# pratikvn/schwarz-lib

Hardware: AMD Instinct MI355X
Metric: RAS iterations/sec + time-to-residual(1e-6), 3D Poisson, 1/2/4/8 subdomains (higher is better)
Workload: dtype f64; 1 GPU; 3D Poisson 256^3, 1 subdomain on 1 MI355X (BASELINE configs[1]); inner_cg_iters=10, precond=jacobi, overlap=2, partition=regular, rows_per_gpu=16777216, nnz_per_gpu=117047296, spmv_variant=0, matrix_format=row-pair coded, cg_flavour=254, exchange=two-sided, all-gathered residual norms

## Files before the change

### schwarz-lib_amd/csrc/spmv_pair.hip

```cpp
#include <hip/hip_runtime.h>

#include <algorithm>
#include <cstdlib>
#include <cstring>
#include <unordered_map>
#include <vector>

#include "device_utils.hpp"
#include "schwz_hip.h"
#include "schwz_internal.hpp"

namespace schwz {

constexpr int kPairPats = 64;
constexpr int kPairEntries = 512;
constexpr int kPairChunk = 8;
constexpr int kPairTableLds = kPairEntries * 16 + kPairEntries * 4 + (kPairEntries / 4) * 4;

__host__ __device__ inline int pair_stride(int lmax, int ch = kPairChunk) { return (lmax + ch - 1) / ch * ch; }

struct __attribute__((aligned(16))) PairVal {
    double a, b;
};
struct __attribute__((aligned(8))) PairMeta {
// ... 421 lines not shown
            } else {
                accumulate(a.x, ra, base, len, safe, s0, s1, own, own_from_gathers);
                if (dual_t) accumulate(a.x2, ra, base, len, safe, t0, t1, unused, false);
            }
        } else {
            plain_row(ra, dual_t, s0, t0);
            if (has_b) plain_row(ra + 1, dual_t, s1, t1);
        }
        if (kWantOwn && !own_from_gathers) {
            own.x = kDir ? dir1(ra) : a.x[ra];
            if (has_b) own.y = kDir ? dir1(ra + 1) : a.x[ra + 1];
        }
        double y0, y1 = 0.0, p0, p1 = 0.0;
        finish(ra, s0, t0, dual_t, own.x, ob0, od0, y0, p0);
        if (has_b) finish(ra + 1, s1, t1, dual_t, own.y, ob1, od1, y1, p1);
        if (MODE == kSpmvCgUpdate) {
            if (has_b) {
                const pvd2 rr = {y0, y1};
                const pvd2 xx = {cgx.x + p0, cgx.y + p1};
                __builtin_nontemporal_store(rr, reinterpret_cast<pvd2 *>(a.cg_r + ra));
                if (a.cg_x) __builtin_nontemporal_store(xx, reinterpret_cast<pvd2 *>(a.cg_x + ra));
            } else {
                a.cg_r[ra] = y0;
                if (a.cg_x) a.cg_x[ra] = cgx.x + p0;
            }
        } else if (kDir) {
            if (has_b)
                __builtin_memcpy(a.y + ra, &own, 16);
            else
                a.y[ra] = own.x;
        } else if (MODE != kSpmvResidNorm && !kDotOnly) {
            if (has_b) {
                const pvd2 yy = {y0, y1};
                if (MODE == kSpmvResidInit || MODE == kSpmvResidDual)
                    __builtin_nontemporal_store(yy, reinterpret_cast<pvd2 *>(a.y + ra));
                else
                    __builtin_memcpy(a.y + ra, &yy, 16);
            } else {
                a.y[ra] = y0;
            }
        }
        if (MODE == kSpmvResidInit || MODE == kSpmvResidDual) {
            if (has_b) {
                const pvd2 pp = {p0, p1};
                __builtin_nontemporal_store(pp, reinterpret_cast<pvd2 *>(a.p + ra));
            } else {
                a.p[ra] = p0;
            }
        }
    }
    if (MODE != kSpmvPlain) {
        const double s0 = block_sum(acc0, red);
        const double s1 = block_sum(acc1, red);
        if (tid == 0) {
            const int stride = a.part_stride ? a.part_stride : (int)gridDim.x;
            a.partials[a.part_offset + blockIdx.x] = s0;
            a.partials[stride + a.part_offset + blockIdx.x] = s1;
        }
        if (MODE == kSpmvResidDual) {
            const double s2v = block_sum(acc2, red);
            if (tid == 0) a.partials[2 * gridDim.x + blockIdx.x] = s2v;
        }
    }
    if (kDir && blockIdx.x == 0 && tid == 0 && !a.sweep) {
        CgState *st = const_cast<CgState *>(a.cg_state);
        st->rho[(a.it + 1) & 1] = cg_rho_new;
        st->rr = cg_rr;
        st->iters = st->iters + 1;
        if (sqrt(cg_rr) <= a.cg_rtol * st->r0) st->stop_iter = 0;
    }
}

#ifndef SCHWZ_WALK_ZEROCOEF
#define SCHWZ_WALK_ZEROCOEF 1
#endif

#ifndef SCHWZ_WALK_HINTS
#define SCHWZ_WALK_HINTS 1
#endif
#ifndef SCHWZ_INIT_PLAIN_STORE
#define SCHWZ_INIT_PLAIN_STORE 1
#endif

template <int NHL, int NH, bool DIAGVEC, bool INIT = false, bool DUAL = false, int RUNS = 8>
__global__ __launch_bounds__(kBlock) void spmv_pair_sweep_kernel(CsrView A, SpmvArgs a)
{
#pragma clang fp contract(off)
    extern __shared__ __attribute__((aligned(16))) char sweep_lds[];
    constexpr int T = NH * kPairRows;
    const int NX = A.sweep_nx;
    double *const own_ring = reinterpret_cast<double *>(sweep_lds);
    double *const halo_ring = own_ring + 4 * T;
    PairVal *const cpv = reinterpret_cast<PairVal *>(halo_ring + 4 * NX);
    int *const cmask = reinterpret_cast<int *>(cpv + A.canon_npat * 9);
    __shared__ double red[4];
    double cg_alpha = 1.0;
    const int tid = threadIdx.x;
    if (!INIT) {
        if (a.it >= a.cg_state->stop_iter) return;
    }
    typedef double pvd2u __attribute__((ext_vector_type(2), aligned(8)));
    const double *const r_in = INIT ? a.b : a.cg_r;
    double *const r_out = INIT ? a.y : (a.cg_r_out ? a.cg_r_out : a.cg_r);
    const pvd2 ring_scale = {a.ring_scale, a.ring_scale};
    auto tables_and_alpha = [&]() {
        for (int i = tid; i < A.canon_npat * 9; i += kBlock) {
            if (SCHWZ_WALK_ZEROCOEF) {
                const int m = A.canon_mask[i / 9], k = i % 9;
                cpv[i] = PairVal{((m >> k) & 1) ? A.canon_val[2 * i] : 0.0, ((m >> (16 + k)) & 1) ? A.canon_val[2 * i + 1] : 0.0};
            } else {
                cpv[i] = PairVal{A.canon_val[2 * i], A.canon_val[2 * i + 1]};
            }
        }
        if (tid < A.canon_npat) cmask[tid] = A.canon_mask[tid];
        if (!INIT) {
            cg_alpha = a.cg_state->rho[a.it & 1] / fold_partials(a.pq_partials, a.pq_nparts, red);
            if (blockIdx.x == 0 && tid == 0 && a.alpha_out) *a.alpha_out = cg_alpha;
        }
        lds_barrier();
    };
    if (blockIdx.x == 0)
        for (int i = (int)gridDim.x + a.part_offset + tid; i < a.part_stride; i += kBlock) {
            a.partials[i] = a.partials[a.part_stride + i] = 0.0;
            if (DUAL) a.partials[2 * a.part_stride + i] = 0.0;
        }
    const int4 sg = A.sweep_seg[blockIdx.x];
    const int64_t PL = A.sweep_pl;
    const int band = sg.x, z0 = sg.y, z1 = sg.z;
    constexpr bool GEN = RUNS == 0;
    const int blen = GEN ? sg.w : T;
    const int64_t gmax = A.ncols - 2;
    double acc0 = 0.0, acc1 = 0.0, acc2 = 0.0;
    typedef const unsigned __attribute__((address_space(4))) *const_words;
    typedef const int __attribute__((address_space(4))) *const_ints;
    if (z0 < z1) {
        const const_ints chain = (const_ints)(uintptr_t)A.chain_plane;
        const const_ints chain_far = (const_ints)(uintptr_t)A.chain_far;
        auto band_row = [&](int z) -> int {
            const int k = chain[z];
            return (k < 0 ? 0 : k) * (int)PL + band * T;
        };
        auto clampg = [&](int g) -> int { return g < 0 ? 0 : (g > (int)gmax ? (int)gmax : g); };
        auto load_own = [&](int base, pvd2 (&reg)[NH]) {
#pragma unroll
            for (int k = 0; k < NH; ++k) __builtin_memcpy(&reg[k], a.x + clampg(base + 2 * (tid + k * kBlock)), 16);
        };
        auto store_own = [&](int z, const pvd2 (&reg)[NH]) {
            double *slot_p = own_ring + (size_t)(z & 3) * T;
#pragma unroll
            for (int k = 0; k < NH; ++k) *reinterpret_cast<pvd2 *>(slot_p + 2 * (tid + k * kBlock)) = ring_scale * reg[k];
        };
        auto load_halo = [&](int base, pvd2 (&reg)[NHL]) {
            const int lo = base - NX, up = base + T;
#pragma unroll
            for (int k = 0; k < NHL; ++k) {
                const int pc = min(tid + k * kBlock, NX - 1);
                const int g = pc < NX / 2 ? lo + 2 * pc : up + 2 * (pc - NX / 2);
                __builtin_memcpy(&reg[k], a.x + clampg(g), 16);
            }
        };
        auto store_halo = [&](int z, const pvd2 (&reg)[NHL]) {
            double *slot_p = halo_ring + (size_t)(z & 1) * 2 * NX;
#pragma unroll
            for (int k = 0; k < NHL; ++k) {
                const int pc = min(tid + k * kBlock, NX - 1);
                *reinterpret_cast<pvd2 *>(slot_p + 2 * pc) = ring_scale * reg[k];
            }
        };
        struct Ahead {
            pvd2 r, d;
            unsigned w[GEN ? 1 : RUNS / 2];
        };
        auto fetch = [&](int base, int h) -> Ahead {
            Ahead f;
            const int row0 = base + h * kPairRows;
            const int ra = GEN ? base + min(h * kPairRows + 2 * tid, blen - 2) : row0 + 2 * tid;
            if (GEN) {
                f.w[0] = A.pair_id[ra >> 1];
            } else {
                const const_words q = (const_words)(uintptr_t)(A.pair_rle + (row0 / kPairRows) * ((RUNS ? RUNS : 8) / 8));
#pragma unroll
                for (int k = 0; k < (GEN ? 1 : RUNS / 2); ++k) f.w[k] = q[k];
            }
            if (SCHWZ_WALK_HINTS)
                f.r = __builtin_nontemporal_load(reinterpret_cast<const pvd2u *>(r_in + ra));
            else
                f.r = *reinterpret_cast<const pvd2u *>(r_in + ra);
            if (DIAGVEC) f.d = __builtin_nontemporal_load(reinterpret_cast<const pvd2 *>(a.dinv + ra));
            return f;
        };
        pvd2 own_a[NH], own_b[NH], hreg[NHL];
        Ahead r_a[NH], r_b[NH];
        int brow[5];
#pragma unroll
        for (int k = 0; k < 5; ++k) brow[k] = band_row(z0 - 1 + k);
        {
            pvd2 first[NH], second[NH];
            load_own(brow[0], first);
            load_own(brow[1], second);
            load_halo(brow[1], hreg);
            load_own(brow[2], own_b);
            load_own(brow[3], own_a);
#pragma unroll
            for (int h = 0; h < NH; ++h) {
                r_a[h] = fetch(brow[1], h);
                r_b[h] = fetch(z0 + 1 < z1 ? brow[2] : brow[1], h);
            }
            tables_and_alpha();
            store_own(z0 - 1, first);
            store_own(z0, second);
        }
        auto step = [&](int z, pvd2 (&own_next)[NH], Ahead (&rr)[NH]) {
            store_own(z + 1, own_next);
            store_halo(z, hreg);
            lds_barrier();
            load_halo(brow[2], hreg);
            load_own(brow[4], own_next);
            const int far = chain_far[z];
            const bool plain_pos = DUAL ? ((const_ints)(uintptr_t)A.chain_dual)[z] == 0 : true;
            const double *cur = own_ring + (size_t)(z & 3) * T;
            const double *prv = own_ring + (size_t)((z + 3) & 3) * T;
            const double *nxt = own_ring + (size_t)((z + 1) & 3) * T;
            const double *hlo = halo_ring + (size_t)(z & 1) * 2 * NX, *hup = hlo + NX;
            const double *fb0 = (far & 3) == 1 ? prv : ((far & 3) == 2 ? nxt : cur);
            const double *fb1 = ((far >> 2) & 3) == 1 ? prv : (((far >> 2) & 3) == 2 ? nxt : cur);
            const double *fa0 = ((far >> 4) & 3) == 1 ? prv : (((far >> 4) & 3) == 2 ? nxt : cur);
            const double *fa1 = ((far >> 6) & 3) == 1 ? prv : (((far >> 6) & 3) == 2 ? nxt : cur);
            const int rbase = z + 2 < z1 ? brow[3] : brow[1];
#pragma unroll
            for (int h = 0; h < NH; ++h) {
                const Ahead f = rr[h];
                const int i0u = h * kPairRows + 2 * tid;
                const bool valid = !GEN || i0u < blen;
                const int i0 = GEN ? min(i0u, blen - 2) : i0u;
                const int ra = brow[1] + i0;
                int pid = GEN ? (int)f.w[0] : (int)((f.w[0] >> 8) & 0xffu);
#pragma unroll
                for (int k = 1; k < RUNS; ++k) {
                    const unsigned e = (f.w[k >> 1] >> ((k & 1) * 16)) & 0xffffu;
                    if ((unsigned)tid >= (e & 0xffu)) pid = (int)(e >> 8);
                }
                const int mask = SCHWZ_WALK_ZEROCOEF ? 0 : cmask[pid];
                pvd2 t[8];
                t[4] = *reinterpret_cast<const pvd2 *>(cur + i0);
                t[3].x = i0 > 0 ? cur[i0 - 1] : hlo[NX - 1];
                t[3].y = t[4].x;
                t[5].x = t[4].y;
                t[5].y = i0 + 2 < T ? cur[i0 + 2] : hup[0];
                t[2] = *reinterpret_cast<const pvd2 *>(i0 >= NX ? cur + (i0 - NX) : hlo + i0);
                t[6] = *reinterpret_cast<const pvd2 *>(i0 + NX < T ? cur + (i0 + NX) : hup + (i0 + NX - T));
                t[0] = *reinterpret_cast<const pvd2 *>(fb0 + i0);
                t[7] = *reinterpret_cast<const pvd2 *>(fa0 + i0);
                double s0 = 0.0, s1 = 0.0;
                auto add = [&](int k, pvd2 tv) {
                    const PairVal v = cpv[pid * 9 + k];
                    const double p0 = v.a * tv.x, p1 = v.b * tv.y;
                    if (SCHWZ_WALK_ZEROCOEF) {
                        s0 += p0;
                        s1 += p1;
                    } else {
                        s0 += ((mask >> k) & 1) ? p0 : 0.0;
                        s1 += ((mask >> (16 + k)) & 1) ? p1 : 0.0;
                    }
                };
                add(0, t[0]);
                if (far & 0x0c) add(1, *reinterpret_cast<const pvd2 *>(fb1 + i0));
#pragma unroll
                for (int k = 2; k < 8; ++k) add(k, t[k]);
                if (far & 0xc0) add(8, *reinterpret_cast<const pvd2 *>(fa1 + i0));
                const double r0 = INIT ? f.r.x - s0 : f.r.x - cg_alpha * s0;
                const double zz0 = a.diag_mode ? (DIAGVEC ? f.d.x : a.diag_uniform) * r0 : r0;
                const double r1 = INIT ? f.r.y - s1 : f.r.y - cg_alpha * s1;
                const double zz1 = a.diag_mode ? (DIAGVEC ? f.d.y : a.diag_uniform) * r1 : r1;
                if (GEN) {
                    const double t00 = r0 * zz0, t01 = r0 * r0, t10 = r1 * zz1, t11 = r1 * r1;
                    acc0 += valid ? t00 : 0.0;
                    acc1 += valid ? t01 : 0.0;
                    acc0 += valid ? t10 : 0.0;
                    acc1 += valid ? t11 : 0.0;
                } else {
                    acc0 += r0 * zz0;
                    acc1 += r0 * r0;
                    acc0 += r1 * zz1;
                    acc1 += r1 * r1;
                }
                if (DUAL) {
                    const double q0 = r0 * r0, q1 = r1 * r1;
                    acc2 += plain_pos ? q0 : 0.0;
                    acc2 += plain_pos ? q1 : 0.0;
                }
                const pvd2 rn = {r0, r1};
                if (SCHWZ_WALK_HINTS && !(INIT && SCHWZ_INIT_PLAIN_STORE))
                    __builtin_nontemporal_store(rn, reinterpret_cast<pvd2 *>(r_out + ra));
                else
                    *reinterpret_cast<pvd2 *>(r_out + ra) = rn;
                rr[h] = fetch(rbase, h);
            }
#pragma unroll
            for (int k = 0; k < 4; ++k) brow[k] = brow[k + 1];
            brow[4] = band_row(z + 4);
        };
        int z = z0;
        for (; z + 1 < z1; z += 2) {
            step(z, own_b, r_a);
            step(z + 1, own_a, r_b);
        }
        if (z < z1) step(z, own_b, r_a);
    } else if (!INIT && blockIdx.x == 0) {
        tables_and_alpha();
    }
    const double s0 = block_sum(acc0, red);
    const double s1 = block_sum(acc1, red);
    if (tid == 0) {
        a.partials[blockIdx.x] = s0;
        a.partials[a.part_stride + blockIdx.x] = s1;
    }
    if (DUAL) {
        const double s2 = block_sum(acc2, red);
        if (tid == 0) a.partials[2 * a.part_stride + blockIdx.x] = s2;
    }
}

#ifndef SCHWZ_DD
#define SCHWZ_DD 7
#endif
template <int NHL, int NH, bool FIRST = false, int RUNS = 8>
__global__ __launch_bounds__(kBlock) void spmv_pair_dirdot_sweep_kernel(CsrView A, SpmvArgs a)
{
#pragma clang fp contract(off)
    extern __shared__ __attribute__((aligned(16))) char sweep_lds[];
    constexpr int T = NH * kPairRows;
    const int NX = A.sweep_nx;
    double *const own_ring = reinterpret_cast<double *>(sweep_lds);
    constexpr int kHaloSlots = (SCHWZ_DD & 2) ? 3 : 2;
    double *const halo_ring = own_ring + 4 * T;
    PairVal *const cpv = reinterpret_cast<PairVal *>(halo_ring + kHaloSlots * NX);
    int *const cmask = reinterpret_cast<int *>(cpv + A.canon_npat * 5);
    __shared__ double red[4];
    if (!FIRST && a.it >= a.cg_state->stop_iter) return;
    double cg_rho_new = 0.0, cg_rr = 0.0, cg_beta = 0.0;
    const int tid = threadIdx.x;
    auto init_fold = [&]() {
        if (FIRST && a.init_fold && blockIdx.x == 0)
            cg_init_state(const_cast<CgState *>(a.cg_state), a.pq_partials, a.pq_nparts, a.cg_rtol, a.norm_sq_out,
                          a.norm_bank, red);
    };
    auto tables_and_beta = [&]() {
        for (int i = tid; i < A.canon_npat * 5; i += kBlock) {
            if (SCHWZ_WALK_ZEROCOEF) {
                const int m = A.canon_sym_mask[i / 5], k = i % 5;
                cpv[i] = PairVal{((m >> k) & 1) ? A.canon_sym_val[2 * i] : 0.0, ((m >> (16 + k)) & 1) ? A.canon_sym_val[2 * i + 1] : 0.0};
            } else {
                cpv[i] = PairVal{A.canon_sym_val[2 * i], A.canon_sym_val[2 * i + 1]};
            }
        }
        if (tid < A.canon_npat) cmask[tid] = A.canon_sym_mask[tid];
        if (!FIRST) {
            cg_rho_new = fold_partials(a.pq_partials, a.pq_nparts, red);
            cg_rr = fold_partials(a.pq_partials + a.pq_nparts, a.pq_nparts, red);
            cg_beta = cg_rho_new / a.cg_state->rho[a.it & 1];
        }
        init_fold();
        lds_barrier();
    };
    if (blockIdx.x == 0)
        for (int i = (int)gridDim.x + a.part_offset + tid; i < a.part_stride; i += kBlock)
            a.partials[i] = a.partials[a.part_stride + i] = 0.0;
    const int4 sg = A.sweep_seg_dir[blockIdx.x];
    const int64_t PL = A.sweep_pl;
    const int band = sg.x, z0 = sg.y, z1 = sg.z;
    constexpr bool GEN = RUNS == 0;
    const int blen = GEN ? sg.w : T;
    const int64_t gmax = A.ncols - 2;
    const pvd2 du = {a.diag_uniform, a.diag_uniform};
    double acc0 = 0.0;
    typedef const unsigned __attribute__((address_space(4))) *const_words;
    typedef const int __attribute__((address_space(4))) *const_ints;
    if (z0 < z1) {
        const const_ints chain = (const_ints)(uintptr_t)A.chain_plane;
        const const_ints chain_far = (const_ints)(uintptr_t)A.chain_far;
        auto band_row = [&](int z) -> int {
            const int k = chain[z];
            return (k < 0 ? 0 : k) * (int)PL + band * T;
        };
        auto clampg = [&](int g) -> int { return g < 0 ? 0 : (g > (int)gmax ? (int)gmax : g); };
        const pvd2 p_scale = {a.p_scale, a.p_scale};
        auto newp = [&](pvd2 rv, pvd2 pv) -> pvd2 {
            const pvd2 zv = a.diag_mode ? du * rv : rv;
            if (FIRST) return zv;
            const pvd2 ps = p_scale * pv;
// ... 119 lines not shown
            const double *prv = own_ring + (size_t)((z + 3) & 3) * T;
            const double *nxt = own_ring + (size_t)((z + 1) & 3) * T;
            const double *hup = halo_ring + (size_t)((SCHWZ_DD & 2) ? hs : (z & 1)) * NX;
            const double *fa0 = ((far >> 4) & 3) == 1 ? prv : (((far >> 4) & 3) == 2 ? nxt : cur);
            const double *fa1 = ((far >> 6) & 3) == 1 ? prv : (((far >> 6) & 3) == 2 ? nxt : cur);
            const int rbase = z + 2 < z1 ? brow[3] : brow[1];
#pragma unroll
            for (int h = 0; h < NH; ++h) {
                const Rle f = rl[h];
                const int i0u = h * kPairRows + 2 * tid;
                const bool valid = !GEN || i0u < blen;
                const int i0 = GEN ? min(i0u, blen - 2) : i0u;
                int pid = GEN ? (int)f.w[0] : (int)((f.w[0] >> 8) & 0xffu);
#pragma unroll
                for (int k = 1; k < RUNS; ++k) {
                    const unsigned e = (f.w[k >> 1] >> ((k & 1) * 16)) & 0xffffu;
                    if ((unsigned)tid >= (e & 0xffu)) pid = (int)(e >> 8);
                }
                const int mask = SCHWZ_WALK_ZEROCOEF ? 0 : cmask[pid];
                pvd2 t[4];
                t[0] = *reinterpret_cast<const pvd2 *>(cur + i0);
                t[1].x = t[0].y;
                t[1].y = i0 + 2 < T ? cur[i0 + 2] : hup[0];
                t[2] = *reinterpret_cast<const pvd2 *>(i0 + NX < T ? cur + (i0 + NX) : hup + (i0 + NX - T));
                t[3] = *reinterpret_cast<const pvd2 *>(fa0 + i0);
                double s0 = 0.0, s1 = 0.0;
                auto add = [&](int k, pvd2 tv) {
                    const PairVal v = cpv[pid * 5 + k];
                    const double p0 = v.a * tv.x, p1 = v.b * tv.y;
                    if (SCHWZ_WALK_ZEROCOEF) {
                        s0 += p0;
                        s1 += p1;
                    } else {
                        s0 += ((mask >> k) & 1) ? p0 : 0.0;
                        s1 += ((mask >> (16 + k)) & 1) ? p1 : 0.0;
                    }
                };
#pragma unroll
                for (int k = 0; k < 4; ++k) add(k, t[k]);
                if (far & 0xc0) add(4, *reinterpret_cast<const pvd2 *>(fa1 + i0));
                if (GEN) {
                    const double u0 = t[0].x * s0, u1 = t[0].y * s1;
                    acc0 += valid ? u0 : 0.0;
                    acc0 += valid ? u1 : 0.0;
                } else {
                    acc0 += t[0].x * s0;
                    acc0 += t[0].y * s1;
                }
                rl[h] = fetch_rle(rbase, h);
            }
#pragma unroll
            for (int k = 0; k < 4; ++k) brow[k] = brow[k + 1];
            brow[4] = band_row(z + 4);
            hs = hs_next;
        };
        int z = z0;
        for (; z + 1 < z1; z += 2) {
            step(z, own_b, rle_a, hreg);
            step(z + 1, own_a, rle_b, hreg_b);
        }
        if (z < z1) step(z, own_b, rle_a, hreg);
    } else if (!FIRST && blockIdx.x == 0) {
        tables_and_beta();
    } else {
        init_fold();
    }
    const double s0 = block_sum(acc0, red);
    if (tid == 0) {
        a.partials[blockIdx.x] = s0;
        a.partials[a.part_stride + blockIdx.x] = 0.0;
    }
    if (!FIRST && blockIdx.x == 0 && tid == 0) {
        CgState *st = const_cast<CgState *>(a.cg_state);
        st->rho[(a.it + 1) & 1] = cg_rho_new;
        st->rr = cg_rr;
        st->iters = st->iters + 1;
        if (sqrt(cg_rr) <= a.cg_rtol * st->r0) st->stop_iter = 0;
    }
}


constexpr size_t kSweepLdsLimit = 96 << 10;

static size_t sweep_update_lds(int64_t T, int64_t nx, int npat)
{
    return (size_t)(4 * T + 4 * nx) * sizeof(double) + (size_t)npat * (9 * 16 + 4);
}

static size_t sweep_dirdot_lds(int64_t T_dir, int64_t nx, int npat)
{
    return (size_t)(4 * T_dir + ((SCHWZ_DD & 2) ? 3 : 2) * nx) * sizeof(double) + (size_t)npat * (5 * 16 + 4);
}

bool pair_sweep_update_ok(const CsrView &A, int grid, int diag_mode)
{
    const int nh = A.sweep_T / kPairRows, nhl = (A.sweep_nx + kBlock - 1) / kBlock;
    return A.pair_single && A.sweep_nslots > 0 && A.ncols < (int64_t(1) << 28) && diag_mode != 2 &&
           A.sweep_nslots + A.sweep_gen_blocks <= grid && (nh == 1 || nh == 2) && nhl <= 4 &&
           sweep_update_lds(A.sweep_T, A.sweep_nx, A.canon_npat) <= kSweepLdsLimit;
}

bool pair_sweep_dirdot_ok(const CsrView &A, int grid, int diag_mode)
{
    const int nh = A.sweep_T_dir / kPairRows, nhl = (A.sweep_nx / 2 + kBlock - 1) / kBlock;
    return pair_sweep_update_ok(A, grid, diag_mode) && A.canon_sym_val && diag_mode != 1 &&
           A.sweep_nslots_dir + A.sweep_gen_blocks <= grid && (nh == 1 || nh == 2 || nh == 4) && nhl <= 2 &&
           sweep_dirdot_lds(A.sweep_T_dir, A.sweep_nx, A.canon_npat) <= kSweepLdsLimit;
}

bool pair_sweep_start_ok(const CsrView &A, int grid)
{
    return A.sweep_gen_blocks == 0 && pair_sweep_dirdot_ok(A, grid, 0);
}

bool pair_sweep_dual_ok(const CsrView &A, int grid)
{
    return pair_sweep_start_ok(A, grid) && A.chain_dual && A.dual_chunks && A.dual_blocks > 0 &&
           A.sweep_nslots + A.dual_blocks <= grid;
}

template <void (*KERNEL)(CsrView, SpmvArgs)>
static bool launch_walk_kernel(int nslots, const CsrView &A, const SpmvArgs &b, size_t lds, hipStream_t s)
{
    static const hipError_t e = hipFuncSetAttribute((const void *)KERNEL, hipFuncAttributeMaxDynamicSharedMemorySize,
                                                    kSweepLdsLimit);
    if (e != hipSuccess || lds > kSweepLdsLimit) return false;
    hipLaunchKernelGGL(KERNEL, dim3(nslots), dim3(kBlock), lds, s, A, b);
    return true;
}

template <int L_, int H_, bool DV, bool INIT, bool DUAL>
static bool launch_sweep_variant(const CsrView &A, const SpmvArgs &b, size_t lds, hipStream_t s)
{
    if (A.sweep_gen_mode) {
        if (DUAL) return false;
        return launch_walk_kernel<spmv_pair_sweep_kernel<L_, H_, DV, INIT, false, 0>>(A.sweep_nslots, A, b, lds, s);
    }
    return A.pair_rle_runs == 16
               ? launch_walk_kernel<spmv_pair_sweep_kernel<L_, H_, DV, INIT, DUAL, 16>>(A.sweep_nslots, A, b, lds, s)
               : launch_walk_kernel<spmv_pair_sweep_kernel<L_, H_, DV, INIT, DUAL, 8>>(A.sweep_nslots, A, b, lds, s);
}

template <bool DV, bool INIT, bool DUAL>
static bool launch_update_walk(const CsrView &A, const SpmvArgs &b, hipStream_t s)
{
    const int nhl = (A.sweep_nx + kBlock - 1) / kBlock, nh = A.sweep_T / kPairRows;
    const size_t lds = sweep_update_lds(A.sweep_T, A.sweep_nx, A.canon_npat);
    if (nh == 1)
        return nhl == 1   ? launch_sweep_variant<1, 1, DV, INIT, DUAL>(A, b, lds, s)
               : nhl == 2 ? launch_sweep_variant<2, 1, DV, INIT, DUAL>(A, b, lds, s)
                          : launch_sweep_variant<4, 1, DV, INIT, DUAL>(A, b, lds, s);
    return nhl == 1   ? launch_sweep_variant<1, 2, DV, INIT, DUAL>(A, b, lds, s)
           : nhl == 2 ? launch_sweep_variant<2, 2, DV, INIT, DUAL>(A, b, lds, s)
                      : launch_sweep_variant<4, 2, DV, INIT, DUAL>(A, b, lds, s);
}

template <int L_, int H_, bool FIRST>
static bool launch_dirdot_variant(const CsrView &A, const SpmvArgs &b, size_t lds, hipStream_t s)
{
    const int nslots = A.sweep_nslots_dir;
    if (A.sweep_gen_mode) return launch_walk_kernel<spmv_pair_dirdot_sweep_kernel<L_, H_, FIRST, 0>>(nslots, A, b, lds, s);
    return A.pair_rle_runs == 16 ? launch_walk_kernel<spmv_pair_dirdot_sweep_kernel<L_, H_, FIRST, 16>>(nslots, A, b, lds, s)
                                 : launch_walk_kernel<spmv_pair_dirdot_sweep_kernel<L_, H_, FIRST, 8>>(nslots, A, b, lds, s);
}

template <bool FIRST>
static bool launch_dirdot_walk(const CsrView &A, const SpmvArgs &b, hipStream_t s)
{
    const int nhl = (A.sweep_nx / 2 + kBlock - 1) / kBlock, nh = A.sweep_T_dir / kPairRows;
    const size_t lds = sweep_dirdot_lds(A.sweep_T_dir, A.sweep_nx, A.canon_npat);
    if (nh == 1)
        return nhl == 1 ? launch_dirdot_variant<1, 1, FIRST>(A, b, lds, s) : launch_dirdot_variant<2, 1, FIRST>(A, b, lds, s);
    if (nh == 2)
        return nhl == 1 ? launch_dirdot_variant<1, 2, FIRST>(A, b, lds, s) : launch_dirdot_variant<2, 2, FIRST>(A, b, lds, s);
    return nhl == 1 ? launch_dirdot_variant<1, 4, FIRST>(A, b, lds, s) : launch_dirdot_variant<2, 4, FIRST>(A, b, lds, s);
}

int launch_spmv_pair(const CsrView &A, int mode, const SpmvArgs &a, int grid, hipStream_t s)
{
    const bool wide = A.ncols >= (int64_t(1) << 28);
    const char *const no_lds = "launch_spmv_pair: the z-sweep kernels cannot have 96 KiB of dynamic LDS on this device";
    if ((mode == kSpmvResidInit || mode == kSpmvResidDual) && a.sweep_init) {
        if (!pair_sweep_start_ok(A, grid) || a.diag_mode == 1 || a.diag_mode == 2 || a.dinv) {
            set_error("launch_spmv_pair: the z-sweep start launch does not apply to this matrix");
            return SCHWZ_ERR_INVALID;
        }
        SpmvArgs b = a;
        b.part_stride = grid;
        b.part_offset = 0;
        const bool with_dual = mode == kSpmvResidDual && a.x2 != nullptr;
        if (with_dual && !pair_sweep_dual_ok(A, grid)) {
            set_error("launch_spmv_pair: the z-sweep dual start launch does not apply to this matrix");
            return SCHWZ_ERR_INVALID;
        }
        if (!(with_dual ? launch_update_walk<false, true, true>(A, b, s) : launch_update_walk<false, true, false>(A, b, s))) {
            set_error(no_lds);
            return SCHWZ_ERR_HIP;
        }
        SCHWZ_HIP_TRY(hipGetLastError());
        if (with_dual) {
            SpmvArgs c;
            c.x = a.x2;
            c.b = a.b;
            c.row_limit = a.row_limit;
            c.sweep = 2;
            c.partials = a.partials + grid;
            c.part_stride = grid;
            c.part_offset = A.sweep_nslots;
            hipLaunchKernelGGL((spmv_pair_kernel<kSpmvResidNorm, false, true>), dim3(A.dual_blocks), dim3(kBlock),
                               kPairTableLds, s, A, c);
            SCHWZ_HIP_TRY(hipGetLastError());
        }
        return SCHWZ_OK;
    }
    if (mode == kSpmvDirDotSym && a.sweep_first) {
        if (!pair_sweep_start_ok(A, grid) || a.diag_mode == 1 || a.diag_mode == 2) {
            set_error("launch_spmv_pair: the z-sweep first-direction launch does not apply to this matrix");
            return SCHWZ_ERR_INVALID;
        }
        CsrView Af = A;
        if (A.sweep_seg_first && A.sweep_nslots_first <= grid) {
            Af.sweep_T_dir = A.sweep_T_first;
            Af.sweep_seg_dir = A.sweep_seg_first;
            Af.sweep_nslots_dir = A.sweep_nslots_first;
        }
        SpmvArgs b = a;
        b.part_stride = grid;
        b.part_offset = 0;
        if (!launch_dirdot_walk<true>(Af, b, s)) {
            set_error(no_lds);
// ... 131 lines not shown
    const int nplanes = (int)(nrows / PL), cpp = (int)(PL / kPairRows);
    auto in_plane = [&](schwz_idx off) { return off == 0 || off == 1 || off == -1 || off == NX || off == -NX; };
    std::vector<std::vector<schwz_idx>> pat_far((size_t)tb.npat);
    std::vector<uint8_t> pat_bad((size_t)tb.npat, 0);
    for (int q = 0; q < tb.npat; ++q) {
        if ((int)tb.len[(size_t)q] > 9) pat_bad[(size_t)q] = 1;
        for (int k = 0; k < (int)tb.len[(size_t)q]; ++k) {
            const schwz_idx off = tb.ent[(size_t)q * tb.lmax + k].off;
            if (in_plane(off)) continue;
            if (off % PL != 0) pat_bad[(size_t)q] = 1;
            pat_far[(size_t)q].push_back(off);
        }
    }
    std::vector<uint8_t> plane_ok((size_t)nplanes, 1);
    std::vector<std::vector<schwz_idx>> plane_far((size_t)nplanes);
    std::vector<std::vector<int>> plane_pats((size_t)nplanes);
    for (int k = 0; k < nplanes; ++k) {
        std::vector<uint8_t> used((size_t)tb.npat, 0);
        if (gen_mode)
            for (int64_t pr = (int64_t)k * PL / 2; pr < (int64_t)(k + 1) * PL / 2; ++pr) used[(size_t)pair_id[(size_t)pr]] = 1;
        for (int c = k * cpp; !gen_mode && c < (k + 1) * cpp && plane_ok[(size_t)k]; ++c) {
            const int R = A->v.pair_rle_runs;
            if (rle[(size_t)c * R] == 0xffffu) {
                plane_ok[(size_t)k] = 0;
                break;
            }
            for (int r = 0; r < R; ++r) used[(size_t)(rle[(size_t)c * R + r] >> 8)] = 1;
        }
        if (!plane_ok[(size_t)k]) continue;
        std::vector<schwz_idx> far;
        for (int q = 0; q < tb.npat; ++q) {
            if (!used[(size_t)q]) continue;
            plane_pats[(size_t)k].push_back(q);
            if (pat_bad[(size_t)q]) plane_ok[(size_t)k] = 0;
            for (schwz_idx f : pat_far[(size_t)q]) far.push_back(f);
        }
        std::sort(far.begin(), far.end());
        far.erase(std::unique(far.begin(), far.end()), far.end());
        int nb = 0, na = 0;
        for (schwz_idx f : far) {
            const int64_t j = k + f / PL;
            if (j < 0 || j >= nplanes) plane_ok[(size_t)k] = 0;
            (f < 0 ? nb : na)++;
        }
        if (far.size() > 2 || nb > 2 || na > 2) plane_ok[(size_t)k] = 0;
        if (plane_ok[(size_t)k]) plane_far[(size_t)k] = far;
    }
    std::vector<std::vector<int>> adj((size_t)nplanes);
    auto link = [&](int x, int y) {
        if (std::find(adj[(size_t)x].begin(), adj[(size_t)x].end(), y) == adj[(size_t)x].end()) adj[(size_t)x].push_back(y);
    };
    for (int k = 0; k < nplanes; ++k)
        for (schwz_idx f : plane_far[(size_t)k]) {
            link(k, (int)(k + f / PL));
            link((int)(k + f / PL), k);
        }
    for (int k = 0; k < nplanes; ++k)
        if (adj[(size_t)k].size() > 2) {
            plane_ok[(size_t)k] = 0;
            for (int j : adj[(size_t)k]) plane_ok[(size_t)j] = 0;
        }
    std::vector<int> chain_plane;
    std::vector<int> pos_of((size_t)nplanes, -1);
    chain_plane.push_back(-1);
    std::vector<uint8_t> seen((size_t)nplanes, 0);
    for (int pass = 0; pass < 2; ++pass)
        for (int k0 = 0; k0 < nplanes; ++k0) {
            if (seen[(size_t)k0] || adj[(size_t)k0].size() > 2) continue;
            if (pass == 0 && adj[(size_t)k0].size() != 1 && !adj[(size_t)k0].empty()) continue;
            int prev = -1, k = k0;
            while (k >= 0 && !seen[(size_t)k] && adj[(size_t)k].size() <= 2) {
                seen[(size_t)k] = 1;
                pos_of[(size_t)k] = (int)chain_plane.size();
                chain_plane.push_back(k);
                int next = -1;
                for (int j : adj[(size_t)k])
                    if (j != prev && !seen[(size_t)j]) next = j;
                prev = k;
                k = next;
            }
            chain_plane.push_back(-1);
        }
    const int npos = (int)chain_plane.size();
    for (int k = 0; k < 4; ++k) chain_plane.push_back(-1);
    std::vector<int> chain_far((size_t)npos + 4, 0);
    std::vector<double> cval((size_t)tb.npat * 18, 0.0), sval((size_t)tb.npat * 10, 0.0);
    std::vector<int> cmsk((size_t)tb.npat, 0), smsk((size_t)tb.npat, 0);
    std::vector<int8_t> pat_slot_set((size_t)tb.npat, 0);
    std::vector<std::vector<int8_t>> pat_slots((size_t)tb.npat);
    bool sym_ok = ts != nullptr && ts->npat == tb.npat;
    for (int p = 0; p < npos; ++p) {
        const int k = chain_plane[(size_t)p];
        if (k < 0 || !plane_ok[(size_t)k]) continue;
        const std::vector<schwz_idx> &far = plane_far[(size_t)k];
        std::vector<schwz_idx> fb, fa;
        for (schwz_idx f : far) (f < 0 ? fb : fa).push_back(f);
        int code = 0;
        bool ok = true;
        auto src_of = [&](schwz_idx f) -> int {
            const int j = (int)(k + f / PL);
            if (pos_of[(size_t)j] == p - 1) return 1;
            if (pos_of[(size_t)j] == p + 1) return 2;
            ok = false;
            return 0;
        };
        for (size_t i = 0; i < fb.size(); ++i) code |= src_of(fb[i]) << (2 * (int)i);
        for (size_t i = 0; i < fa.size(); ++i) code |= src_of(fa[i]) << (4 + 2 * (int)i);
        for (int q : plane_pats[(size_t)k]) {
            std::vector<int8_t> slots;
            for (int e = 0; e < (int)tb.len[(size_t)q] && ok; ++e) {
                const schwz_idx off = tb.ent[(size_t)q * tb.lmax + e].off;
                int slot = -1;
                if (off == -NX) slot = 2;
                else if (off == -1) slot = 3;
                else if (off == 0) slot = 4;
                else if (off == 1) slot = 5;
                else if (off == NX) slot = 6;
                else {
                    for (size_t i = 0; i < fb.size(); ++i)
                        if (fb[i] == off) slot = (int)i;
                    for (size_t i = 0; i < fa.size(); ++i)
                        if (fa[i] == off) slot = 7 + (int)i;
                }
                if (slot < 0) ok = false;
                slots.push_back((int8_t)slot);
            }
            if (!ok) break;
            if (pat_slot_set[(size_t)q] && pat_slots[(size_t)q] != slots) ok = false;
            if (!ok) break;
            pat_slot_set[(size_t)q] = 1;
            pat_slots[(size_t)q] = slots;
        }
        if (!ok) {
            plane_ok[(size_t)k] = 0;
            continue;
        }
        chain_far[(size_t)p] = code;
    }
    for (int q = 0; q < tb.npat; ++q) {
        if (!pat_slot_set[(size_t)q]) continue;
        for (int e = 0; e < (int)tb.len[(size_t)q]; ++e) {
            const PairEntryH &en = tb.ent[(size_t)q * tb.lmax + e];
            const int slot = pat_slots[(size_t)q][(size_t)e];
            std::memcpy(&cval[((size_t)q * 9 + slot) * 2], &en.va, 8);
            std::memcpy(&cval[((size_t)q * 9 + slot) * 2 + 1], &en.vb, 8);
            cmsk[(size_t)q] |= (en.flags & 1) << slot;
            cmsk[(size_t)q] |= ((en.flags >> 1) & 1) << (16 + slot);
        }
        if (sym_ok) {
            for (int e = 0; e < (int)ts->len[(size_t)q]; ++e) {
                const PairEntryH &en = ts->ent[(size_t)q * ts->lmax + e];
                int slot = -1;
                for (int f = 0; f < (int)tb.len[(size_t)q]; ++f)
                    if (tb.ent[(size_t)q * tb.lmax + f].off == en.off) slot = pat_slots[(size_t)q][(size_t)f] - 4;
                if (slot < 0 || slot > 4) {
                    sym_ok = false;
                    break;
                }
                std::memcpy(&sval[((size_t)q * 5 + slot) * 2], &en.va, 8);
                std::memcpy(&sval[((size_t)q * 5 + slot) * 2 + 1], &en.vb, 8);
                smsk[(size_t)q] |= (en.flags & 1) << slot;
                smsk[(size_t)q] |= ((en.flags >> 1) & 1) << (16 + slot);
            }
        }
    }
    const char *t_env = std::getenv("SCHWZ_SWEEP_T"), *l_env = std::getenv("SCHWZ_SWEEP_L");
    int T = t_env ? std::atoi(t_env) : ((NX >= 512 || (two_d && PL % 1024 == 0)) ? 1024 : 512);
    if (T != 512 && T != 1024) T = 512;
    if (PL % T && !gen_mode) T = 512;
    if (gen_mode && PL < T) T = 512;
    auto walk_lds = [&](int t) { return sweep_update_lds(t, NX, tb.npat); };
    if (walk_lds(T) > kSweepLdsLimit && T == 1024 && PL % 512 == 0) T = 512;
    if (walk_lds(T) > kSweepLdsLimit) return no_walk("ring and pattern tables exceed 96 KiB of LDS");
    if (NX > T) return no_walk("x line longer than a band");
    const int bands = (int)((PL + T - 1) / T);
    const int grid = (int)((std::min<int64_t>(ntiles, kMaxGrid) + kXcds - 1) / kXcds) * kXcds;
    struct Run { int p0, p1; };
    std::vector<Run> runs;
    int64_t steps = 0;
    for (int p = 0; p < npos;) {
        const int k = chain_plane[(size_t)p];
        if (k < 0 || !plane_ok[(size_t)k]) {
            ++p;
            continue;
        }
        int e = p;
        while (e < npos && chain_plane[(size_t)e] >= 0 && plane_ok[(size_t)chain_plane[(size_t)e]]) ++e;
        if (e - p >= 2) {
            runs.push_back({p, e});
            steps += (int64_t)(e - p) * bands;
        }
        p = e;
    }
    if (runs.empty()) return no_walk("no chain of two or more walkable planes");
    std::vector<uint8_t> covered((size_t)nchunks, 0);
    std::vector<schwz_idx> gen;
    if (gen_mode) {
        int64_t walked = 0;
        for (const Run &r : runs) walked += r.p1 - r.p0;
        if (walked != nplanes) return no_walk("planes that are not whole chunks: some plane cannot be walked (and nothing can be left to the chunk launches)");
    } else {
        for (const Run &r : runs)
            for (int p = r.p0; p < r.p1; ++p)
                for (int c = 0; c < cpp; ++c) covered[(size_t)chain_plane[(size_t)p] * cpp + c] = 1;
        for (int c = 0; c < nchunks; ++c)
            if (!covered[(size_t)c]) gen.push_back(c);
    }
    int cus = 256;
    {
        int dev = 0;
        hipDeviceProp_t prop;
        if (hipGetDevice(&dev) == hipSuccess && hipGetDeviceProperties(&prop, dev) == hipSuccess && prop.multiProcessorCount > 0)
            cus = prop.multiProcessorCount;
    }
    const int per_cu = T == 1024 ? 2 : 3;
    int L = l_env ? std::atoi(l_env) : (int)std::max<int64_t>(8, (steps + per_cu * cus - 1) / (per_cu * cus));
    if (L < 2) L = 16;
    auto count = [&](int len) {
        int64_t n = 0;
        for (const Run &r : runs) n += (int64_t)((r.p1 - r.p0 + len - 1) / len) * bands;
        return n;
    };
    const int seg_slots = (int)((count(L) + kXcds - 1) / kXcds * kXcds) + kXcds;
    const int gen_blocks = (int)std::min<int64_t>((int64_t)gen.size(), std::max(256, std::min(1024, grid - seg_slots)));
    while (count(L) + kXcds > grid - gen_blocks && L < (1 << 20)) L += 4;
    struct Seg { int band, p0, p1; };
    auto make_slots = [&](int Tq, int Lq) -> std::vector<int4> {
        const int bands_q = (int)((PL + Tq - 1) / Tq);
        std::vector<Seg> segs;
        for (const Run &r : runs) {
            const int nseg = (r.p1 - r.p0 + Lq - 1) / Lq, len = (r.p1 - r.p0 + nseg - 1) / nseg;
            for (int b = 0; b < bands_q; ++b)
                for (int p = r.p0; p < r.p1; p += len) segs.push_back({b, p, std::min(p + len, r.p1)});
        }
        std::stable_sort(segs.begin(), segs.end(), [](const Seg &x, const Seg &y) { return x.p0 != y.p0 ? x.p0 < y.p0 : x.band < y.band; });
        std::vector<std::vector<int4>> per_xcd(kXcds);
        for (const Seg &sgm : segs) {
            int4 v;
            v.x = sgm.band;
            v.y = sgm.p0;
            v.z = sgm.p1;
            v.w = (int)std::min<int64_t>(Tq, PL - (int64_t)sgm.band * Tq);
            size_t x;
            if (bands_q >= 2 * kXcds) {
                x = (size_t)((int64_t)sgm.band * kXcds / bands_q);
            } else {
                x = 0;
                for (size_t k = 1; k < (size_t)kXcds; ++k)
                    if (per_xcd[k].size() < per_xcd[x].size()) x = k;
            }
            per_xcd[x].push_back(v);
        }
        size_t depth = 0;
        for (const auto &l : per_xcd) depth = std::max(depth, l.size());
// ... 601 lines not shown
```

Before: 633.2 subdomain-iter/s.

## Stream sweep walk operands into LDS with async global_load_lds pipelining

Replaces the register-staged plane loads in the sweep SpMV walk with direct global-to-LDS DMA (global_load_lds_dwordx4) into multi-slot rings for the own plane, halo and residual input, prefetched D planes ahead with vmcnt-based waits. This is meant to hide global-memory latency and free the VGPRs that held the prefetched planes. In exchange it uses more LDS, which may lower occupancy or force a smaller band size, and it relies on inline asm that manipulates the M0 register and on vmcnt accounting being correct. The diagonal-vector and generic paths keep the old scheme.

```diff
diff --git a/schwarz-lib_amd/csrc/spmv_pair.hip b/schwarz-lib_amd/csrc/spmv_pair.hip
--- a/schwarz-lib_amd/csrc/spmv_pair.hip
+++ b/schwarz-lib_amd/csrc/spmv_pair.hip
@@ -527,6 +527,41 @@
 #define SCHWZ_INIT_PLAIN_STORE 1
 #endif
 
+#ifndef SCHWZ_WALK_DEPTH_UPDATE
+#define SCHWZ_WALK_DEPTH_UPDATE 2
+#endif
+#ifndef SCHWZ_WALK_DEPTH_START
+#define SCHWZ_WALK_DEPTH_START 2
+#endif
+constexpr int kWalkDepthMax = SCHWZ_WALK_DEPTH_UPDATE > SCHWZ_WALK_DEPTH_START ? SCHWZ_WALK_DEPTH_UPDATE : SCHWZ_WALK_DEPTH_START;
+static_assert(SCHWZ_WALK_DEPTH_UPDATE == 0 || (SCHWZ_WALK_DEPTH_UPDATE >= 2 && SCHWZ_WALK_DEPTH_UPDATE <= 6), "update walk depth: 0 or 2 .. 6");
+static_assert(SCHWZ_WALK_DEPTH_START == 0 || (SCHWZ_WALK_DEPTH_START >= 2 && SCHWZ_WALK_DEPTH_START <= 6), "start walk depth: 0 or 2 .. 6");
+constexpr int kChainLookAhead = 4 > kWalkDepthMax + 1 ? 4 : kWalkDepthMax + 1;
+
+constexpr int walk_depth(bool init, bool diagvec, bool gen)
+{
+    return (diagvec || gen) ? 0 : (init ? SCHWZ_WALK_DEPTH_START : SCHWZ_WALK_DEPTH_UPDATE);
+}
+
+template <bool NT>
+__device__ __forceinline__ void glds16(const void *gsrc, unsigned lds_dst)
+{
+    unsigned keep;
+    if (NT)
+        asm volatile("s_mov_b32 %0, m0\n\ts_mov_b32 m0, %2\n\ts_nop 0\n\tglobal_load_lds_dwordx4 %1, off nt\n\ts_mov_b32 m0, %0"
+                     : "=&s"(keep) : "v"(gsrc), "s"(lds_dst) : "memory");
+    else
+        asm volatile("s_mov_b32 %0, m0\n\ts_mov_b32 m0, %2\n\ts_nop 0\n\tglobal_load_lds_dwordx4 %1, off\n\ts_mov_b32 m0, %0"
+                     : "=&s"(keep) : "v"(gsrc), "s"(lds_dst) : "memory");
+}
+
+template <int N>
+__device__ __forceinline__ void walk_wait_vm()
+{
+    static_assert(N >= 0 && N < 64, "vmcnt is a 6-bit count");
+    asm volatile("s_waitcnt vmcnt(%0)" ::"n"(N) : "memory");
+}
+
 template <int NHL, int NH, bool DIAGVEC, bool INIT = false, bool DUAL = false, int RUNS = 8>
 __global__ __launch_bounds__(kBlock) void spmv_pair_sweep_kernel(CsrView A, SpmvArgs a)
 {
@@ -534,9 +569,12 @@
     extern __shared__ __attribute__((aligned(16))) char sweep_lds[];
     constexpr int T = NH * kPairRows;
     const int NX = A.sweep_nx;
+    constexpr int D = walk_depth(INIT, DIAGVEC, RUNS == 0);
+    constexpr int kHaloSlot = NHL * kBlock * 2;
     double *const own_ring = reinterpret_cast<double *>(sweep_lds);
-    double *const halo_ring = own_ring + 4 * T;
-    PairVal *const cpv = reinterpret_cast<PairVal *>(halo_ring + 4 * NX);
+    double *const r_ring = own_ring + (D + 2) * T;
+    double *const halo_ring = D ? r_ring + D * T : own_ring + 4 * T;
+    PairVal *const cpv = reinterpret_cast<PairVal *>(D ? halo_ring + D * kHaloSlot : halo_ring + 4 * NX);
     int *const cmask = reinterpret_cast<int *>(cpv + A.canon_npat * 9);
     __shared__ double red[4];
     double cg_alpha = 1.0;
@@ -562,6 +600,7 @@
             cg_alpha = a.cg_state->rho[a.it & 1] / fold_partials(a.pq_partials, a.pq_nparts, red);
             if (blockIdx.x == 0 && tid == 0 && a.alpha_out) *a.alpha_out = cg_alpha;
         }
+        if (D) walk_wait_vm<0>();
         lds_barrier();
     };
     if (blockIdx.x == 0)
@@ -627,130 +666,224 @@
 #pragma unroll
                 for (int k = 0; k < (GEN ? 1 : RUNS / 2); ++k) f.w[k] = q[k];
             }
-            if (SCHWZ_WALK_HINTS)
+            if (D) {
+                f.r = pvd2{0.0, 0.0};
+            } else if (SCHWZ_WALK_HINTS) {
                 f.r = __builtin_nontemporal_load(reinterpret_cast<const pvd2u *>(r_in + ra));
-            else
+            } else {
                 f.r = *reinterpret_cast<const pvd2u *>(r_in + ra);
+            }
             if (DIAGVEC) f.d = __builtin_nontemporal_load(reinterpret_cast<const pvd2 *>(a.dinv + ra));
             return f;
         };
-        pvd2 own_a[NH], own_b[NH], hreg[NHL];
-        Ahead r_a[NH], r_b[NH];
-        int brow[5];
-#pragma unroll
-        for (int k = 0; k < 5; ++k) brow[k] = band_row(z0 - 1 + k);
-        {
-            pvd2 first[NH], second[NH];
-            load_own(brow[0], first);
-            load_own(brow[1], second);
-            load_halo(brow[1], hreg);
-            load_own(brow[2], own_b);
-            load_own(brow[3], own_a);
-#pragma unroll
-            for (int h = 0; h < NH; ++h) {
-                r_a[h] = fetch(brow[1], h);
-                r_b[h] = fetch(z0 + 1 < z1 ? brow[2] : brow[1], h);
-            }
-            tables_and_alpha();
-            store_own(z0 - 1, first);
-            store_own(z0, second);
-        }
-        auto step = [&](int z, pvd2 (&own_next)[NH], Ahead (&rr)[NH]) {
-            store_own(z + 1, own_next);
-            store_halo(z, hreg);
-            lds_barrier();
-            load_halo(brow[2], hreg);
-            load_own(brow[4], own_next);
-            const int far = chain_far[z];
-            const bool plain_pos = DUAL ? ((const_ints)(uintptr_t)A.chain_dual)[z] == 0 : true;
-            const double *cur = own_ring + (size_t)(z & 3) * T;
-            const double *prv = own_ring + (size_t)((z + 3) & 3) * T;
-            const double *nxt = own_ring + (size_t)((z + 1) & 3) * T;
-            const double *hlo = halo_ring + (size_t)(z & 1) * 2 * NX, *hup = hlo + NX;
+        auto opd2 = [&](const double *q) -> pvd2 {
+            const pvd2 v = *reinterpret_cast<const pvd2 *>(q);
+            return D ? ring_scale * v : v;
+        };
+        auto opd1 = [&](const double *q) -> double { return D ? a.ring_scale * *q : *q; };
+        auto pair_rows = [&](int h, const Ahead &f, pvd2 rv, int row, const double *cur, const double *prv, const double *nxt,
+                             const double *hlo, const double *hup, int far, bool plain_pos) {
             const double *fb0 = (far & 3) == 1 ? prv : ((far & 3) == 2 ? nxt : cur);
             const double *fb1 = ((far >> 2) & 3) == 1 ? prv : (((far >> 2) & 3) == 2 ? nxt : cur);
             const double *fa0 = ((far >> 4) & 3) == 1 ? prv : (((far >> 4) & 3) == 2 ? nxt : cur);
             const double *fa1 = ((far >> 6) & 3) == 1 ? prv : (((far >> 6) & 3) == 2 ? nxt : cur);
-            const int rbase = z + 2 < z1 ? brow[3] : brow[1];
+            const int i0u = h * kPairRows + 2 * tid;
+            const bool valid = !GEN || i0u < blen;
+            const int i0 = GEN ? min(i0u, blen - 2) : i0u;
+            const int ra = row + i0;
+            int pid = GEN ? (int)f.w[0] : (int)((f.w[0] >> 8) & 0xffu);
+#pragma unroll
+            for (int k = 1; k < RUNS; ++k) {
+                const unsigned e = (f.w[k >> 1] >> ((k & 1) * 16)) & 0xffffu;
+                if ((unsigned)tid >= (e & 0xffu)) pid = (int)(e >> 8);
+            }
+            const int mask = SCHWZ_WALK_ZEROCOEF ? 0 : cmask[pid];
+            pvd2 t[8];
+            t[4] = opd2(cur + i0);
+            t[3].x = opd1(i0 > 0 ? cur + (i0 - 1) : hlo + (NX - 1));
+            t[3].y = t[4].x;
+            t[5].x = t[4].y;
+            t[5].y = opd1(i0 + 2 < T ? cur + (i0 + 2) : hup);
+            t[2] = opd2(i0 >= NX ? cur + (i0 - NX) : hlo + i0);
+            t[6] = opd2(i0 + NX < T ? cur + (i0 + NX) : hup + (i0 + NX - T));
+            t[0] = opd2(fb0 + i0);
+            t[7] = opd2(fa0 + i0);
+            double s0 = 0.0, s1 = 0.0;
+            auto add = [&](int k, pvd2 tv) {
+                const PairVal v = cpv[pid * 9 + k];
+                const double p0 = v.a * tv.x, p1 = v.b * tv.y;
+                if (SCHWZ_WALK_ZEROCOEF) {
+                    s0 += p0;
+                    s1 += p1;
+                } else {
+                    s0 += ((mask >> k) & 1) ? p0 : 0.0;
+                    s1 += ((mask >> (16 + k)) & 1) ? p1 : 0.0;
+                }
+            };
+            add(0, t[0]);
+            if (far & 0x0c) add(1, opd2(fb1 + i0));
+#pragma unroll
+            for (int k = 2; k < 8; ++k) add(k, t[k]);
+            if (far & 0xc0) add(8, opd2(fa1 + i0));
+            const double r0 = INIT ? rv.x - s0 : rv.x - cg_alpha * s0;
+            const double zz0 = a.diag_mode ? (DIAGVEC ? f.d.x : a.diag_uniform) * r0 : r0;
+            const double r1 = INIT ? rv.y - s1 : rv.y - cg_alpha * s1;
+            const double zz1 = a.diag_mode ? (DIAGVEC ? f.d.y : a.diag_uniform) * r1 : r1;
+            if (GEN) {
+                const double t00 = r0 * zz0, t01 = r0 * r0, t10 = r1 * zz1, t11 = r1 * r1;
+                acc0 += valid ? t00 : 0.0;
+                acc1 += valid ? t01 : 0.0;
+                acc0 += valid ? t10 : 0.0;
+                acc1 += valid ? t11 : 0.0;
+            } else {
+                acc0 += r0 * zz0;
+                acc1 += r0 * r0;
+                acc0 += r1 * zz1;
+                acc1 += r1 * r1;
+            }
+            if (DUAL) {
+                const double q0 = r0 * r0, q1 = r1 * r1;
+                acc2 += plain_pos ? q0 : 0.0;
+                acc2 += plain_pos ? q1 : 0.0;
+            }
+            const pvd2 rn = {r0, r1};
+            if (SCHWZ_WALK_HINTS && !(INIT && SCHWZ_INIT_PLAIN_STORE))
+                __builtin_nontemporal_store(rn, reinterpret_cast<pvd2 *>(r_out + ra));
+            else
+                *reinterpret_cast<pvd2 *>(r_out + ra) = rn;
+        };
+        if constexpr (D == 0) {
+            pvd2 own_a[NH], own_b[NH], hreg[NHL];
+            Ahead r_a[NH], r_b[NH];
+            int brow[5];
+#pragma unroll
+            for (int k = 0; k < 5; ++k) brow[k] = band_row(z0 - 1 + k);
+            {
+                pvd2 first[NH], second[NH];
+                load_own(brow[0], first);
+                load_own(brow[1], second);
+                load_halo(brow[1], hreg);
+                load_own(brow[2], own_b);
+                load_own(brow[3], own_a);
+#pragma unroll
+                for (int h = 0; h < NH; ++h) {
+                    r_a[h] = fetch(brow[1], h);
+                    r_b[h] = fetch(z0 + 1 < z1 ? brow[2] : brow[1], h);
+                }
+                tables_and_alpha();
+                store_own(z0 - 1, first);
+                store_own(z0, second);
+            }
+            auto step = [&](int z, pvd2 (&own_next)[NH], Ahead (&rr)[NH]) {
+                store_own(z + 1, own_next);
+                store_halo(z, hreg);
+                lds_barrier();
+                load_halo(brow[2], hreg);
+                load_own(brow[4], own_next);
+                const int far = chain_far[z];
+                const bool plain_pos = DUAL ? ((const_ints)(uintptr_t)A.chain_dual)[z] == 0 : true;
+                const double *cur = own_ring + (size_t)(z & 3) * T;
+                const double *prv = own_ring + (size_t)((z + 3) & 3) * T;
+                const double *nxt = own_ring + (size_t)((z + 1) & 3) * T;
+                const double *hlo = halo_ring + (size_t)(z & 1) * 2 * NX, *hup = hlo + NX;
+                const int rbase = z + 2 < z1 ? brow[3] : brow[1];
+#pragma unroll
+                for (int h = 0; h < NH; ++h) {
+                    pair_rows(h, rr[h], rr[h].r, brow[1], cur, prv, nxt, hlo, hup, far, plain_pos);
+                    rr[h] = fetch(rbase, h);
+                }
+#pragma unroll
+                for (int k = 0; k < 4; ++k) brow[k] = brow[k + 1];
+                brow[4] = band_row(z + 4);
+            };
+            int z = z0;
+            for (; z + 1 < z1; z += 2) {
+                step(z, own_b, r_a);
+                step(z + 1, own_a, r_b);
+            }
+            if (z < z1) step(z, own_b, r_a);
+        } else {
+            typedef __attribute__((address_space(3))) char *lds_bytes;
+            const unsigned wave_off = (unsigned)__builtin_amdgcn_readfirstlane(tid >> 6) * 1024u;
+            const unsigned own_lds = (unsigned)(uintptr_t)(lds_bytes)own_ring + wave_off;
+            const unsigned r_lds = (unsigned)(uintptr_t)(lds_bytes)r_ring + wave_off;
+            const unsigned halo_lds = (unsigned)(uintptr_t)(lds_bytes)halo_ring + wave_off;
+            auto dma_own = [&](int base, int slot) {
+#pragma unroll
+                for (int k = 0; k < NH; ++k)
+                    glds16<false>(a.x + clampg(base + 2 * (tid + k * kBlock)), own_lds + (unsigned)(slot * T * 8 + k * kBlock * 16));
+            };
+            auto dma_halo = [&](int base, int slot) {
+                const int lo = base - NX, up = base + T;
+#pragma unroll
+                for (int k = 0; k < NHL; ++k) {
+                    const int pc = min(tid + k * kBlock, NX - 1);
+                    const int g = pc < NX / 2 ? lo + 2 * pc : up + 2 * (pc - NX / 2);
+                    glds16<false>(a.x + clampg(g), halo_lds + (unsigned)(slot * kHaloSlot * 8 + k * kBlock * 16));
+                }
+            };
+            auto dma_r = [&](int base, int slot) {
+#pragma unroll
+                for (int h = 0; h < NH; ++h)
+                    glds16<SCHWZ_WALK_HINTS != 0>(r_in + base + h * kPairRows + 2 * tid, r_lds + (unsigned)(slot * T * 8 + h * kBlock * 16));
+            };
+            constexpr int kGroup = 2 * NH + NHL;
+            constexpr int kInFlight = NH + (D - 2) * (kGroup + NH);
+            Ahead r_a[NH], r_b[NH];
+            int brow[D + 2];
+#pragma unroll
+            for (int k = 0; k < D + 2; ++k) brow[k] = band_row(z0 - 1 + k);
+            dma_own(brow[0], 0);
+            dma_own(brow[1], 1);
+#pragma unroll
+            for (int j = 1; j < D; ++j) {
+                dma_own(brow[j + 1], j + 1);
+                dma_halo(brow[j], j - 1);
+                dma_r(z0 + j - 1 < z1 ? brow[j] : brow[1], j - 1);
+            }
 #pragma unroll
             for (int h = 0; h < NH; ++h) {
-                const Ahead f = rr[h];
-                const int i0u = h * kPairRows + 2 * tid;
-                const bool valid = !GEN || i0u < blen;
-                const int i0 = GEN ? min(i0u, blen - 2) : i0u;
-                const int ra = brow[1] + i0;
-                int pid = GEN ? (int)f.w[0] : (int)((f.w[0] >> 8) & 0xffu);
-#pragma unroll
-                for (int k = 1; k < RUNS; ++k) {
-                    const unsigned e = (f.w[k >> 1] >> ((k & 1) * 16)) & 0xffffu;
-                    if ((unsigned)tid >= (e & 0xffu)) pid = (int)(e >> 8);
-                }
-                const int mask = SCHWZ_WALK_ZEROCOEF ? 0 : cmask[pid];
-                pvd2 t[8];
-                t[4] = *reinterpret_cast<const pvd2 *>(cur + i0);
-                t[3].x = i0 > 0 ? cur[i0 - 1] : hlo[NX - 1];
-                t[3].y = t[4].x;
-                t[5].x = t[4].y;
-                t[5].y = i0 + 2 < T ? cur[i0 + 2] : hup[0];
-                t[2] = *reinterpret_cast<const pvd2 *>(i0 >= NX ? cur + (i0 - NX) : hlo + i0);
-                t[6] = *reinterpret_cast<const pvd2 *>(i0 + NX < T ? cur + (i0 + NX) : hup + (i0 + NX - T));
-                t[0] = *reinterpret_cast<const pvd2 *>(fb0 + i0);
-                t[7] = *reinterpret_cast<const pvd2 *>(fa0 + i0);
-                double s0 = 0.0, s1 = 0.0;
-                auto add = [&](int k, pvd2 tv) {
-                    const PairVal v = cpv[pid * 9 + k];
-                    const double p0 = v.a * tv.x, p1 = v.b * tv.y;
-                    if (SCHWZ_WALK_ZEROCOEF) {
-                        s0 += p0;
-                        s1 += p1;
-                    } else {
-                        s0 += ((mask >> k) & 1) ? p0 : 0.0;
-                        s1 += ((mask >> (16 + k)) & 1) ? p1 : 0.0;
-                    }
-                };
-                add(0, t[0]);
-                if (far & 0x0c) add(1, *reinterpret_cast<const pvd2 *>(fb1 + i0));
-#pragma unroll
-                for (int k = 2; k < 8; ++k) add(k, t[k]);
-                if (far & 0xc0) add(8, *reinterpret_cast<const pvd2 *>(fa1 + i0));
-                const double r0 = INIT ? f.r.x - s0 : f.r.x - cg_alpha * s0;
-                const double zz0 = a.diag_mode ? (DIAGVEC ? f.d.x : a.diag_uniform) * r0 : r0;
-                const double r1 = INIT ? f.r.y - s1 : f.r.y - cg_alpha * s1;
-                const double zz1 = a.diag_mode ? (DIAGVEC ? f.d.y : a.diag_uniform) * r1 : r1;
-                if (GEN) {
-                    const double t00 = r0 * zz0, t01 = r0 * r0, t10 = r1 * zz1, t11 = r1 * r1;
-                    acc0 += valid ? t00 : 0.0;
-                    acc1 += valid ? t01 : 0.0;
-                    acc0 += valid ? t10 : 0.0;
-                    acc1 += valid ? t11 : 0.0;
-                } else {
-                    acc0 += r0 * zz0;
-                    acc1 += r0 * r0;
-                    acc0 += r1 * zz1;
-                    acc1 += r1 * r1;
-                }
-                if (DUAL) {
-                    const double q0 = r0 * r0, q1 = r1 * r1;
-                    acc2 += plain_pos ? q0 : 0.0;
-                    acc2 += plain_pos ? q1 : 0.0;
-                }
-                const pvd2 rn = {r0, r1};
-                if (SCHWZ_WALK_HINTS && !(INIT && SCHWZ_INIT_PLAIN_STORE))
-                    __builtin_nontemporal_store(rn, reinterpret_cast<pvd2 *>(r_out + ra));
-                else
-                    *reinterpret_cast<pvd2 *>(r_out + ra) = rn;
-                rr[h] = fetch(rbase, h);
-            }
-#pragma unroll
-            for (int k = 0; k < 4; ++k) brow[k] = brow[k + 1];
-            brow[4] = band_row(z + 4);
-        };
-        int z = z0;
-        for (; z + 1 < z1; z += 2) {
-            step(z, own_b, r_a);
-            step(z + 1, own_a, r_b);
-        }
-        if (z < z1) step(z, own_b, r_a);
+                r_a[h] = fetch(brow[1], h);
+                r_b[h] = fetch(z0 + 1 < z1 ? brow[2] : brow[1], h);
+            }
+            tables_and_alpha();
+            int so = 0, sh = 0;
+            auto step = [&](int z, Ahead (&rr)[NH]) {
+                walk_wait_vm<kInFlight>();
+                lds_barrier();
+                const int so_free = so == 0 ? D + 1 : so - 1, sh_free = sh == 0 ? D - 1 : sh - 1;
+                dma_own(brow[D + 1], so_free);
+                dma_halo(brow[D], sh_free);
+                dma_r(z + D - 1 < z1 ? brow[D] : brow[1], sh_free);
+                const int far = chain_far[z];
+                const bool plain_pos = DUAL ? ((const_ints)(uintptr_t)A.chain_dual)[z] == 0 : true;
+                const int sc = so == D + 1 ? 0 : so + 1, sn = sc == D + 1 ? 0 : sc + 1;
+                const double *prv = own_ring + (size_t)so * T;
+                const double *cur = own_ring + (size_t)sc * T;
+                const double *nxt = own_ring + (size_t)sn * T;
+                const double *hlo = halo_ring + (size_t)sh * kHaloSlot, *hup = hlo + NX;
+                const double *rcur = r_ring + (size_t)sh * T;
+                const int rbase = z + 2 < z1 ? brow[3] : brow[1];
+#pragma unroll
+                for (int h = 0; h < NH; ++h) {
+                    const pvd2 rv = *reinterpret_cast<const pvd2 *>(rcur + h * kPairRows + 2 * tid);
+                    pair_rows(h, rr[h], rv, brow[1], cur, prv, nxt, hlo, hup, far, plain_pos);
+                    rr[h] = fetch(rbase, h);
+                }
+#pragma unroll
+                for (int k = 0; k < D + 1; ++k) brow[k] = brow[k + 1];
+                brow[D + 1] = band_row(z + 1 + D);
+                so = sc;
+                sh = sh == D - 1 ? 0 : sh + 1;
+            };
+            int z = z0;
+            for (; z + 1 < z1; z += 2) {
+                step(z, r_a);
+                step(z + 1, r_b);
+            }
+            if (z < z1) step(z, r_a);
+            walk_wait_vm<0>();
+        }
     } else if (!INIT && blockIdx.x == 0) {
         tables_and_alpha();
     }
@@ -1036,10 +1169,14 @@
 
 constexpr size_t kSweepLdsLimit = 96 << 10;
 
-static size_t sweep_update_lds(int64_t T, int64_t nx, int npat)
+static size_t sweep_update_lds(int64_t T, int64_t nx, int npat, int depth)
 {
-    return (size_t)(4 * T + 4 * nx) * sizeof(double) + (size_t)npat * (9 * 16 + 4);
-}
+    const int64_t nhl = (nx + kBlock - 1) / kBlock;
+    const int64_t ring = depth ? (2 * depth + 2) * T + depth * nhl * kBlock * 2 : 4 * T + 4 * nx;
+    return (size_t)ring * sizeof(double) + (size_t)npat * (9 * 16 + 4);
+}
+
+static int plan_walk_depth(bool gen_mode) { return gen_mode ? 0 : kWalkDepthMax; }
 
 static size_t sweep_dirdot_lds(int64_t T_dir, int64_t nx, int npat)
 {
@@ -1051,7 +1188,7 @@
     const int nh = A.sweep_T / kPairRows, nhl = (A.sweep_nx + kBlock - 1) / kBlock;
     return A.pair_single && A.sweep_nslots > 0 && A.ncols < (int64_t(1) << 28) && diag_mode != 2 &&
            A.sweep_nslots + A.sweep_gen_blocks <= grid && (nh == 1 || nh == 2) && nhl <= 4 &&
-           sweep_update_lds(A.sweep_T, A.sweep_nx, A.canon_npat) <= kSweepLdsLimit;
+           sweep_update_lds(A.sweep_T, A.sweep_nx, A.canon_npat, plan_walk_depth(A.sweep_gen_mode)) <= kSweepLdsLimit;
 }
 
 bool pair_sweep_dirdot_ok(const CsrView &A, int grid, int diag_mode)
@@ -1099,7 +1236,7 @@
 static bool launch_update_walk(const CsrView &A, const SpmvArgs &b, hipStream_t s)
 {
     const int nhl = (A.sweep_nx + kBlock - 1) / kBlock, nh = A.sweep_T / kPairRows;
-    const size_t lds = sweep_update_lds(A.sweep_T, A.sweep_nx, A.canon_npat);
+    const size_t lds = sweep_update_lds(A.sweep_T, A.sweep_nx, A.canon_npat, walk_depth(INIT, DV, A.sweep_gen_mode));
     if (nh == 1)
         return nhl == 1   ? launch_sweep_variant<1, 1, DV, INIT, DUAL>(A, b, lds, s)
                : nhl == 2 ? launch_sweep_variant<2, 1, DV, INIT, DUAL>(A, b, lds, s)
@@ -1397,8 +1534,8 @@
             chain_plane.push_back(-1);
         }
     const int npos = (int)chain_plane.size();
-    for (int k = 0; k < 4; ++k) chain_plane.push_back(-1);
-    std::vector<int> chain_far((size_t)npos + 4, 0);
+    for (int k = 0; k < kChainLookAhead; ++k) chain_plane.push_back(-1);
+    std::vector<int> chain_far((size_t)npos + kChainLookAhead, 0);
     std::vector<double> cval((size_t)tb.npat * 18, 0.0), sval((size_t)tb.npat * 10, 0.0);
     std::vector<int> cmsk((size_t)tb.npat, 0), smsk((size_t)tb.npat, 0);
     std::vector<int8_t> pat_slot_set((size_t)tb.npat, 0);
@@ -1484,7 +1621,7 @@
     if (T != 512 && T != 1024) T = 512;
     if (PL % T && !gen_mode) T = 512;
     if (gen_mode && PL < T) T = 512;
-    auto walk_lds = [&](int t) { return sweep_update_lds(t, NX, tb.npat); };
+    auto walk_lds = [&](int t) { return sweep_update_lds(t, NX, tb.npat, plan_walk_depth(gen_mode)); };
     if (walk_lds(T) > kSweepLdsLimit && T == 1024 && PL % 512 == 0) T = 512;
     if (walk_lds(T) > kSweepLdsLimit) return no_walk("ring and pattern tables exceed 96 KiB of LDS");
     if (NX > T) return no_walk("x line longer than a band");
```

New measurement: 635.6 subdomain-iter/s, median of 6. No clear change (+0.4%).
